# pierric/smart-chess-rust

Hardware: AMD Instinct MI355X
Metric: MCTS simulations/sec (whole node), self-play rollout=180, at 1/2/4/8 MI355X (higher is better)
Workload: dtype bf16

## Files before the change

### smart-chess-rust_amd/csrc/nn_tower32.hpp

```cpp
#pragma once
#include <type_traits>

#include "nn_kernels.hpp"

namespace scnn {

typedef __attribute__((ext_vector_type(16))) float f32x16;
typedef __attribute__((ext_vector_type(8))) int i32x8;

struct PrecBF16 {
    static constexpr bool FP8 = false;
    static constexpr int EB = 2;
    static constexpr int KS = 16;
    static constexpr int FB = 16;
    typedef bf16x8 frag;
};
struct PrecFP8 {
    static constexpr bool FP8 = true;
    static constexpr int EB = 1;
    static constexpr int KS = 64;
    static constexpr int FB = 32;
    typedef i32x8 frag;
};
template <class P>
constexpr int pix_stride(int channels) { return channels * P::EB + 16; }

template <class P>
__device__ __forceinline__ typename P::frag lds_frag_p(int byte_off) {
    if constexpr (P::FP8) {
        typedef __attribute__((ext_vector_type(4))) int i32x4;
        const i32x4 a = *reinterpret_cast<const i32x4*>(g_smem + byte_off), b = *reinterpret_cast<const i32x4*>(g_smem + byte_off + 16);
        return i32x8{a[0], a[1], a[2], a[3], b[0], b[1], b[2], b[3]};
    } else {
        return lds_frag(byte_off);
    }
}
template <class P>
__device__ __forceinline__ typename P::frag wload_p(__amdgpu_buffer_rsrc_t rsrc, int voff, int ct, int soff) {
    if constexpr (P::FP8) {
        const bf16x8 a = wload(rsrc, voff + ct * 2048, soff), b = wload(rsrc, voff + ct * 2048 + 1024, soff);
        typedef __attribute__((ext_vector_type(4))) int i32x4;
        const i32x4 x = __builtin_bit_cast(i32x4, a), y = __builtin_bit_cast(i32x4, b);
        return i32x8{x[0], x[1], x[2], x[3], y[0], y[1], y[2], y[3]};
    } else {
        return wload(rsrc, voff + ct * 1024, soff);
    }
}
template <class P>
__device__ __forceinline__ f32x16 mma_p(const typename P::frag& a, const typename P::frag& b, const f32x16& c, int scale_a) {
    if constexpr (P::FP8) return __builtin_amdgcn_mfma_scale_f32_32x32x64_f8f6f4(a, b, c, 0, 0, 0, scale_a, 0, 127);
    else return __builtin_amdgcn_mfma_f32_32x32x16_bf16(a, b, c, 0, 0, 0);
}
__device__ __forceinline__ uint32_t pk_fp8x4(float a, float b, float c, float d) {
    int w = __builtin_amdgcn_cvt_pk_fp8_f32(a, b, 0, false);
    return (uint32_t)__builtin_amdgcn_cvt_pk_fp8_f32(c, d, w, true);
}

__device__ inline int gpix2board(int pt, int i) {
    const bool inA = (i < 4) || (i >= 12 && i < 16) || (i >= 20 && i < 28);
    const int a = inA ? (i < 4 ? i : (i < 16 ? i - 8 : i - 12)) : (i < 12 ? i - 4 : (i < 20 ? i - 8 : i - 16));
    return ((2 * pt + (inA ? 0 : 1) + 4 * (a >> 3)) << 3) | (a & 7);
}

typedef float f32x2 __attribute__((ext_vector_type(2)));
typedef __bf16 bf16pair __attribute__((ext_vector_type(2)));
typedef short s16x2 __attribute__((ext_vector_type(2)));
template <typename V>
__device__ __forceinline__ f32x2 pair(const V& v, int k) { return f32x2{v[k], v[k + 1]}; }
__device__ __forceinline__ f32x2 splat(float x) { return f32x2{x, x}; }
__device__ __forceinline__ uint32_t pk_bf16(f32x2 y) { return __builtin_bit_cast(uint32_t, __builtin_convertvector(y, bf16pair)); }
__device__ __forceinline__ uint32_t pk_bf16_relu(f32x2 y) {
    s16x2 s = __builtin_bit_cast(s16x2, __builtin_convertvector(y, bf16pair));
    return __builtin_bit_cast(uint32_t, __builtin_elementwise_max(s, s16x2{0, 0}));
}

template <class P, bool RELU>
__device__ __forceinline__ void store4(int byte_off_row, int chan, f32x2 lo, f32x2 hi) {
    if constexpr (P::FP8) {
        const float l = RELU ? 0.f : -448.f;
        *reinterpret_cast<uint32_t*>(g_smem + byte_off_row + chan) =
            pk_fp8x4(__builtin_amdgcn_fmed3f(lo.x, l, 448.f), __builtin_amdgcn_fmed3f(lo.y, l, 448.f),
                     __builtin_amdgcn_fmed3f(hi.x, l, 448.f), __builtin_amdgcn_fmed3f(hi.y, l, 448.f));
    } else {
        *reinterpret_cast<uint2*>(g_smem + byte_off_row + chan * 2) =
            RELU ? make_uint2(pk_bf16_relu(lo), pk_bf16_relu(hi)) : make_uint2(pk_bf16(lo), pk_bf16(hi));
    }
}

template <int CT>
__device__ __forceinline__ int chan32(int wave, int ct, int g, int h) { return wave * (32 * CT) + ct * 32 + 8 * g + 4 * h; }

template <int CT>
struct ChP {
    f32x4 v[CT][4];
};
template <int CT>
__device__ __forceinline__ void ch_load(ChP<CT>& P, const float* __restrict__ p, int wave, int h) {
#pragma unroll
    for (int ct = 0; ct < CT; ct++)
#pragma unroll
        for (int g = 0; g < 4; g++) P.v[ct][g] = *reinterpret_cast<const f32x4*>(p + chan32<CT>(wave, ct, g, h));
}
template <int CT>
__device__ __forceinline__ void ch_load_lds(ChP<CT>& P, int byte_off, int wave, int h) {
#pragma unroll
    for (int ct = 0; ct < CT; ct++)
#pragma unroll
        for (int g = 0; g < 4; g++) P.v[ct][g] = *reinterpret_cast<const f32x4*>(g_smem + byte_off + chan32<CT>(wave, ct, g, h) * 4);
}
template <int CT>
__device__ __forceinline__ void acc_init(f32x16 (&acc)[CT][2], const ChP<CT>& B) {
#pragma unroll
    for (int ct = 0; ct < CT; ct++)
#pragma unroll
        for (int pt = 0; pt < 2; pt++)
#pragma unroll
            for (int r = 0; r < 16; r++) acc[ct][pt][r] = B.v[ct][r >> 2][r & 3];
}

#ifndef SC_T32_AB
#define SC_T32_AB 4
#endif
template <class P, int CIN, int TAPS, int CT, int TILES, int PSB, int RS, int TPI, bool PRE, int AB = SC_T32_AB>
__device__ __forceinline__ void conv_mma32(int xoff, const bf16_t* __restrict__ Wp, int wave_u, int lane, const int (&px)[2],
                                           f32x16 (&acc)[CT][2], typename P::frag (&bq)[RS][CT], int next_first, const int (&sa)[CT]) {
    typedef typename P::frag frag;
    constexpr int KPT = CIN / P::KS;
    constexpr int SPG = KPT * TPI;
    constexpr int NG = TAPS / TPI;
    constexpr int TB = 64 * P::FB;
    constexpr int SBB = TILES * TB;
    constexpr int KSB = P::KS * P::EB;
    constexpr int PD = RS - 1, AD = AB - 1;
    static_assert(TAPS % TPI == 0 && SPG % RS == 0 && PD < SPG, "bad ring / tap-group geometry");
    static_assert(SPG % AB == 0 && AD <= SPG, "bad image buffer geometry");
    const __amdgpu_buffer_rsrc_t rsrc = __builtin_amdgcn_make_buffer_rsrc(
        const_cast<bf16_t*>(Wp) + (size_t)wave_u * CT * (TB / 2), 0, 0x7fffffff, 0x00020000);
    const int voff = lane * 16;
    auto toffb = [](int t) { return (TAPS == 9) ? ((((t * 11) >> 5) - 1) * 10 + (t - 3 * ((t * 11) >> 5)) - 1) * PSB : 0; };
    frag xq[AB][2];
    int wcur = 0;
    int pc[TPI][2];
#pragma unroll
    for (int tl = 0; tl < TPI; tl++)
#pragma unroll
        for (int pt = 0; pt < 2; pt++) pc[tl][pt] = xoff + px[pt] + toffb(tl);
    if (!PRE) {
#pragma unroll
        for (int st = 0; st < PD; st++)
#pragma unroll
            for (int ct = 0; ct < CT; ct++) bq[st][ct] = wload_p<P>(rsrc, voff, ct, st * SBB);
    }
#pragma unroll
    for (int v = 0; v < AD; v++)
#pragma unroll
        for (int pt = 0; pt < 2; pt++) xq[v][pt] = lds_frag_p<P>(pc[v / KPT][pt] + (v % KPT) * KSB);
#pragma unroll 1
    for (int j = 0; j < NG; j++) {
        const int tn = (j + 1 == NG) ? 0 : j + 1;
        const int wnext = (j == NG - 1) ? next_first : tn * (SPG * SBB);
        int pn[TPI][2];
#pragma unroll
        for (int tl = 0; tl < TPI; tl++)
#pragma unroll
            for (int pt = 0; pt < 2; pt++) pn[tl][pt] = xoff + px[pt] + toffb(tn * TPI + tl);
#pragma unroll
        for (int u = 0; u < SPG; u++) {
            const int slot = u % RS;
#pragma unroll
            for (int ct = 0; ct < CT; ct++)
                bq[(slot + PD) % RS][ct] = (u + PD < SPG) ? wload_p<P>(rsrc, voff, ct, wcur + (u + PD) * SBB)
                                                          : wload_p<P>(rsrc, voff, ct, wnext + (u + PD - SPG) * SBB);
#pragma unroll
            for (int pt = 0; pt < 2; pt++) {
                const int v = u + AD;
                xq[v % AB][pt] = (v < SPG) ? lds_frag_p<P>(pc[v / KPT][pt] + (v % KPT) * KSB)
                                           : lds_frag_p<P>(pn[(v - SPG) / KPT][pt] + ((v - SPG) % KPT) * KSB);
            }
#pragma unroll
            for (int ct = 0; ct < CT; ct++)
#pragma unroll
                for (int pt = 0; pt < 2; pt++)
                    acc[ct][pt] = mma_p<P>(bq[slot][ct], xq[u % AB][pt], acc[ct][pt], sa[ct]);
#pragma unroll
            for (int m = 0; m < 2 * CT; m++) {
                __builtin_amdgcn_sched_group_barrier(0x008, 1, 0);
                if (P::FP8) {
                    __builtin_amdgcn_sched_group_barrier(0x100, CT == 1 ? 2 : 1, 0);
                    __builtin_amdgcn_sched_group_barrier(0x020, 1, 0);
                } else if (CT == 1) {
                    __builtin_amdgcn_sched_group_barrier(0x100, 1, 0);
                    if (m == 0) __builtin_amdgcn_sched_group_barrier(0x020, 1, 0);
                } else {
                    if ((m & 1) == 0)
                        __builtin_amdgcn_sched_group_barrier(0x100, 1, 0);
                    else
                        __builtin_amdgcn_sched_group_barrier(0x020, 1, 0);
                }
            }
            __builtin_amdgcn_sched_barrier(0);
        }
        wcur = wnext;
#pragma unroll
        for (int tl = 0; tl < TPI; tl++)
#pragma unroll
            for (int pt = 0; pt < 2; pt++) pc[tl][pt] = pn[tl][pt];
    }
}

struct LnStat {
    float rstd[2], nm[2];
};
template <int CT>
__device__ inline void ln_reduce(const f32x16 (&acc)[CT][2], LnStat& L, int count, int wave, int lane, float* s_stat2,
                                 int& parity, int& bad) {
    float2* st = reinterpret_cast<float2*>(s_stat2) + (parity & 1) * 256;
    parity ^= 1;
    const int i = lane & 31;
    float s[2], q[2];
#pragma unroll
    for (int pt = 0; pt < 2; pt++) {
        f32x2 a2 = {0.f, 0.f}, b2 = {0.f, 0.f};
#pragma unroll
        for (int ct = 0; ct < CT; ct++)
#pragma unroll
            for (int r = 0; r < 16; r += 2) {
                const f32x2 v = pair(acc[ct][pt], r);
                a2 += v;
                b2 = v * v + b2;
            }
        s[pt] = a2.x + a2.y;
        q[pt] = b2.x + b2.y;
    }
    {
        const auto rs = __builtin_amdgcn_permlane32_swap(__float_as_uint(s[0]), __float_as_uint(s[1]), false, false);
        const auto rq = __builtin_amdgcn_permlane32_swap(__float_as_uint(q[0]), __float_as_uint(q[1]), false, false);
        st[wave * 64 + lane] = make_float2(__uint_as_float(rs[0]) + __uint_as_float(rs[1]), __uint_as_float(rq[0]) + __uint_as_float(rq[1]));
    }
    __syncthreads();
    const float inv = 1.0f / (float)count;
#pragma unroll
    for (int pt = 0; pt < 2; pt++) {
        const int gp = pt * 32 + i;
        float2 a0 = st[gp], a1 = st[64 + gp], a2 = st[128 + gp], a3 = st[192 + gp];
        float S = (a0.x + a1.x) + (a2.x + a3.x);
        float Q = (a0.y + a1.y) + (a2.y + a3.y);
        float mean = S * inv;
        float var = Q * inv - mean * mean;
        bad |= (var != var) ? 1 : 0;
        var = fmaxf(var, 0.f);
        L.rstd[pt] = __frsqrt_rn(var + 1e-6f);
        L.nm[pt] = -mean * L.rstd[pt];
    }
}
template <int CT>
__device__ __forceinline__ void ln_apply(f32x16 (&acc)[CT][2], const LnStat& L, const ChP<CT>& G, const ChP<CT>& E, bool relu) {
#pragma unroll
    for (int pt = 0; pt < 2; pt++)
#pragma unroll
        for (int ct = 0; ct < CT; ct++)
#pragma unroll
            for (int r = 0; r < 16; r += 2) {
                const f32x2 t = pair(acc[ct][pt], r) * splat(L.rstd[pt]) + splat(L.nm[pt]);
                const f32x2 y = t * pair(G.v[ct][r >> 2], r & 3) + pair(E.v[ct][r >> 2], r & 3);
                acc[ct][pt][r] = relu ? fmaxf(y.x, 0.f) : y.x;
                acc[ct][pt][r + 1] = relu ? fmaxf(y.y, 0.f) : y.y;
            }
}
template <class P, int CT>
__device__ __forceinline__ void ln_apply_relu_store(const f32x16 (&acc)[CT][2], const LnStat& L, const ChP<CT>& G, const ChP<CT>& E,
                                                    const int (&pixbase)[2], int wave, int h) {
#pragma unroll
    for (int ct = 0; ct < CT; ct++)
#pragma unroll
        for (int pt = 0; pt < 2; pt++)
#pragma unroll
            for (int g = 0; g < 4; g++) {
                f32x2 y[2];
#pragma unroll
                for (int hf = 0; hf < 2; hf++) {
                    const f32x2 t = pair(acc[ct][pt], 4 * g + 2 * hf) * splat(L.rstd[pt]) + splat(L.nm[pt]);
                    y[hf] = t * pair(G.v[ct][g], 2 * hf) + pair(E.v[ct][g], 2 * hf);
                }
                store4<P, true>(pixbase[pt], chan32<CT>(wave, ct, g, h), y[0], y[1]);
            }
}
template <int CT>
__device__ inline void layernorm32(f32x16 (&acc)[CT][2], const ChP<CT>& G, const ChP<CT>& E, int count, bool relu, int wave,
                                   int lane, float* s_stat2, int& parity, int& bad) {
    LnStat L;
    ln_reduce<CT>(acc, L, count, wave, lane, s_stat2, parity, bad);
    ln_apply<CT>(acc, L, G, E, relu);
}

template <class P, int CT>
__device__ inline void store_image32(const f32x16 (&acc)[CT][2], const int (&pixbase)[2], int wave, int h) {
#pragma unroll
    for (int ct = 0; ct < CT; ct++)
#pragma unroll
        for (int pt = 0; pt < 2; pt++)
#pragma unroll
            for (int g = 0; g < 4; g++)
                store4<P, false>(pixbase[pt], chan32<CT>(wave, ct, g, h), pair(acc[ct][pt], 4 * g), pair(acc[ct][pt], 4 * g + 2));
}

template <int CTRL>
__device__ __forceinline__ float dpp_mov(float x) { return dpp_f<CTRL>(x); }
template <int LVL>
__device__ __forceinline__ float pool_xchg(float x) {
    if constexpr (LVL == 1) return dpp_mov<0x140>(x);
    else if constexpr (LVL == 2) return dpp_mov<0x141>(x);
    else if constexpr (LVL == 3) return dpp_mov<0x4E>(x);
    else return dpp_mov<0xB1>(x);
}
template <int NV, int W, int LVL>
__device__ __forceinline__ void pool_level(float (&v)[NV], int lane) {
    if constexpr (LVL < 5) {
        if constexpr (W >= 1) {
            if constexpr (LVL == 0) {
#pragma unroll
                for (int t = 0; t < W; t++) {
                    const auto r = __builtin_amdgcn_permlane16_swap(__float_as_uint(v[t]), __float_as_uint(v[t + W]), false, false);
                    v[t] = __uint_as_float(r[0]) + __uint_as_float(r[1]);
                }
            } else {
                const bool hi = (lane & (16 >> LVL)) != 0;
#pragma unroll
                for (int t = 0; t < W; t++) {
                    float send = hi ? v[t] : v[t + W], keep = hi ? v[t + W] : v[t];
                    v[t] = keep + pool_xchg<LVL>(send);
                }
            }
            pool_level<NV, W / 2, LVL + 1>(v, lane);
        } else {
            v[0] += pool_xchg<LVL>(v[0]);
            pool_level<NV, 0, LVL + 1>(v, lane);
        }
    }
}

template <class P, int CT, int TILES, int RS>
__device__ __forceinline__ void ring_fill(typename P::frag (&bq)[RS][CT], const bf16_t* __restrict__ Wp, int wave_u, int lane) {
    constexpr int TB = 64 * P::FB;
    const __amdgpu_buffer_rsrc_t rsrc = __builtin_amdgcn_make_buffer_rsrc(
        const_cast<bf16_t*>(Wp) + (size_t)wave_u * CT * (TB / 2), 0, 0x7fffffff, 0x00020000);
#pragma unroll
    for (int st = 0; st < RS - 1; st++)
#pragma unroll
        for (int ct = 0; ct < CT; ct++) bq[st][ct] = wload_p<P>(rsrc, lane * 16, ct, st * TILES * TB);
}
template <class P, int CT>
__device__ __forceinline__ void scale_load(int (&sa)[CT], const NetDev& net, int conv_idx, int wave, int lane) {
#pragma unroll
    for (int ct = 0; ct < CT; ct++)
        sa[ct] = P::FP8 ? __builtin_bit_cast(int, net.wf[net.f_scales + (size_t)((conv_idx * 8 + wave * CT + ct) * 64 + lane)]) : 127;
}

template <class P, int C>
struct TowerLds {
    static constexpr int IMG_BYTES = (100 * pix_stride<P>(C) > 4864 * 4) ? 100 * pix_stride<P>(C) : 4864 * 4;
    static constexpr int HIMG_BYTES = 64 * pix_stride<P>(HEAD);
    static constexpr int HIMG = IMG_BYTES;
    static constexpr int STAT = HIMG + HIMG_BYTES;
    static constexpr int VEC = STAT + 4096;
    static constexpr int SCL = VEC + 3072;
    static constexpr int RED = SCL + 1024;
    static constexpr int PAR = RED + 64;
    static constexpr int TOTAL = PAR + 15 * C * 2;
    static_assert(4864 * 4 <= IMG_BYTES, "policy logits (and the softmax pass that reads 19 x 256 of them) must fit in the image area");
    static_assert(IMG_BYTES % 16 == 0 && HIMG_BYTES % 16 == 0, "LDS regions must stay 16-byte aligned");
    static_assert(6 * HEAD * 4 + 3 * POL_PAD * 4 <= TOTAL - VEC, "head parameters must fit in the staging area");
};
static_assert(TowerLds<PrecBF16, 128>::TOTAL == 73088 && TowerLds<PrecBF16, 256>::TOTAL == 102528, "bf16 tower LDS");
static_assert(TowerLds<PrecFP8, 128>::TOTAL == 48960 && TowerLds<PrecFP8, 256>::TOTAL == 60544, "fp8 tower LDS");

struct NoPre {
    __device__ __forceinline__ bool operator()(int) const { return true; }
};
struct Fc1Hand {
    typedef __attribute__((ext_vector_type(4))) unsigned int u32x4;
    Fc1W w;
    uint32_t early;
    int have_a;
    u32x4 a[8];
};
struct NoHand {};
template <class P, int C, int RS, int TPI, int AB = SC_T32_AB, class Pre = NoPre, class Hand = NoHand>
__device__ __forceinline__ bool tower_body(const TowerArgs& A, const int pos, const int8_t* planes_lds, Pre pre, Hand& fhr) {
    constexpr bool FUSED = !std::is_same<Pre, NoPre>::value;
    constexpr bool HAND = std::is_same<Hand, Fc1Hand>::value;
    Hand* const fh = &fhr;
    typedef typename P::frag frag;
    constexpr int CT = C / 128;
    constexpr int TILES = C / 32;
    constexpr int PSB = pix_stride<P>(C);
    constexpr int HPSB = pix_stride<P>(HEAD);
    constexpr int EB = P::EB;
    constexpr int HRS = P::FP8 ? C / 64 : 8, HAB = P::FP8 ? 2 : SC_T32_AB;
    constexpr int H2RS = P::FP8 ? HEAD / 64 : 16, H2AB = P::FP8 ? 2 : SC_T32_AB;
    constexpr int NTW = C / 64;
    typedef TowerLds<P, C> Lds;
    unsigned char* smem = g_smem;
    float* s_stat = reinterpret_cast<float*>(smem + Lds::STAT);
    float* s_scl = reinterpret_cast<float*>(smem + Lds::SCL);
    float* s_red = reinterpret_cast<float*>(smem + Lds::RED);
    bf16_t* s_xb = reinterpret_cast<bf16_t*>(smem + Lds::VEC);
    float* s_z = reinterpret_cast<float*>(smem);

    const int tid = threadIdx.x, lane = tid & 63;
    const int wave = __builtin_amdgcn_readfirstlane(tid >> 6);
    const int i32 = lane & 31, h = lane >> 5;
    const NetDev& net = A.net;
    const int bp[2] = {gpix2board(0, i32), gpix2board(1, i32)};
    const int pixbase[2] = {hidx(bp[0]) * PSB, hidx(bp[1]) * PSB};
    const int px[2] = {pixbase[0] + h * P::FB, pixbase[1] + h * P::FB};

    frag ring[RS][CT];
    int sa[CT], san[CT];
    scale_load<P, CT>(sa, net, 0, wave, lane);
    scale_load<P, CT>(san, net, net.n_blocks > 0 ? 1 : 1 + 2 * net.n_blocks, wave, lane);
    ChP<CT> Bn;
    const int p_in = tid >> 2, q_in = tid & 3;
    uint32_t win[7];
    if (!FUSED && !planes_lds) {
        const uint32_t* src = reinterpret_cast<const uint32_t*>(A.boards + (size_t)pos * 7168 + p_in * 112 + q_in * 28);
#pragma unroll
        for (int k = 0; k < 7; k++) win[k] = src[k];
    }
    static_assert(C <= 256, "one parameter vector per thread");
    f32x4 spv = f32x4{0.f, 0.f, 0.f, 0.f};
    if (tid < 3 * C / 4) spv = *reinterpret_cast<const f32x4*>(net.wf + net.f_stem + tid * 4);
    else if (tid < C) spv = *reinterpret_cast<const f32x4*>(net.wf + net.f_blocks + (tid - 3 * C / 4) * 4);
    if (!FUSED || wave != 0) ring_fill<P, CT, TILES, RS>(ring, net.wb + net.o_stem, wave, lane);
    __builtin_amdgcn_sched_barrier(0);
    if constexpr (FUSED) {
        __shared__ int s_go;
        if (wave <= 1) {
            const bool go = pre(wave);
            if (wave == 0 && lane == 0) s_go = go ? 1 : 0;
            if (wave == 0) ring_fill<P, CT, TILES, RS>(ring, net.wb + net.o_stem, wave, lane);
        } else {
            uint4* z = reinterpret_cast<uint4*>(smem);
            for (int k = tid - 128; k < 100 * PSB / 16; k += 128) z[k] = make_uint4(0, 0, 0, 0);
        }
        __syncthreads();
        if (!s_go) return false;
    } else {
        uint4* z = reinterpret_cast<uint4*>(smem);
        for (int k = tid; k < 100 * PSB / 16; k += 256) z[k] = make_uint4(0, 0, 0, 0);
        __syncthreads();
    }
    if (FUSED || planes_lds) {
        const uint32_t* src = reinterpret_cast<const uint32_t*>(planes_lds + p_in * 112 + q_in * 28);
#pragma unroll
        for (int k = 0; k < 7; k++) win[k] = src[k];
    }
    {
        uint32_t* dst = reinterpret_cast<uint32_t*>(smem + hidx(p_in) * PSB + q_in * 28 * EB);
#pragma unroll
        for (int k = 0; k < 7; k++) {
            const uint32_t w = win[k];
            float v[4];
#pragma unroll
            for (int b = 0; b < 4; b++) v[b] = (float)(int8_t)((w >> (8 * b)) & 0xff);
            if constexpr (P::FP8) {
                dst[k] = pk_fp8x4(v[0], v[1], v[2], v[3]);
            } else {
                dst[2 * k] = pk_bf16(f32x2{v[0], v[1]});
                dst[2 * k + 1] = pk_bf16(f32x2{v[2], v[3]});
            }
        }
        if (tid < C) *reinterpret_cast<f32x4*>(g_smem + Lds::PAR + tid * 16) = spv;
    }
    __syncthreads();

    f32x16 acc[CT][2];
    int ln_parity = 0;
    int bad = 0;
    f32x16 res[CT][2];
    auto store_res = [&]() {
#pragma unroll
        for (int ct = 0; ct < CT; ct++)
#pragma unroll
            for (int pt = 0; pt < 2; pt++) res[ct][pt] = acc[ct][pt];
    };
    auto dump = [&](int stage) {
        if constexpr (FUSED) return;
        if (A.dbg && A.dbg_stage == stage) {
#pragma unroll
            for (int ct = 0; ct < CT; ct++)
#pragma unroll
                for (int pt = 0; pt < 2; pt++)
#pragma unroll
                    for (int r = 0; r < 16; r++)
                        A.dbg[((size_t)pos * 64 + bp[pt]) * C + chan32<CT>(wave, ct, r >> 2, h) + (r & 3)] = acc[ct][pt][r];
        }
    };

    {
        ch_load_lds<CT>(Bn, Lds::PAR, wave, h);
        acc_init<CT>(acc, Bn);
        const bf16_t* w0 = net.wb + net.o_stem;
        conv_mma32<P, 128, 9, CT, TILES, PSB, RS, TPI, true, AB>(0, w0, wave, lane, px, acc, ring, (int)((net.wb + net.o_blocks) - w0) * 2, sa);
        ChP<CT> G, E;
        ch_load_lds<CT>(G, Lds::PAR + C * 4, wave, h);
        ch_load_lds<CT>(E, Lds::PAR + 2 * C * 4, wave, h);
        ch_load_lds<CT>(Bn, Lds::PAR + 3 * C * 4, wave, h);
        layernorm32<CT>(acc, G, E, C, true, wave, lane, s_stat, ln_parity, bad);
    }
    store_res();
    store_image32<P, CT>(acc, pixbase, wave, h);
    __syncthreads();
    dump(0);
    const int head_conv0 = 1 + 2 * net.n_blocks;

#pragma unroll 1
    for (int b = 0; b < net.n_blocks; b++) {
        const bf16_t* wb = net.wb + net.o_blocks + (size_t)b * net.blk_stride_b;
        const float* wf = net.wf + net.f_blocks + (size_t)b * net.blk_stride_f;
        constexpr int NT1 = C / 32;
        constexpr int NTW1 = NT1 / 4;
        constexpr int PAR_V4 = 15 * C / 8;
        constexpr int NPV = (PAR_V4 + 255) / 256;
        constexpr int P_G1 = Lds::PAR, P_E1 = Lds::PAR + 4 * C, P_B2 = Lds::PAR + 8 * C, P_G2 = Lds::PAR + 12 * C, P_E2 = Lds::PAR + 16 * C;
        constexpr int P_SB1 = Lds::PAR + 20 * C, P_SB2 = Lds::PAR + 22 * C, P_BN = Lds::PAR + 26 * C;
        f32x4 pv[NPV];
#pragma unroll
        for (int k = 0; k < NPV; k++)
            if (tid + 256 * k < PAR_V4) pv[k] = *reinterpret_cast<const f32x4*>(wf + C + (size_t)(tid + 256 * k) * 4);
        __builtin_amdgcn_sched_barrier(0);
        acc_init<CT>(acc, Bn);
#pragma unroll
        for (int ct = 0; ct < CT; ct++) sa[ct] = san[ct];
        scale_load<P, CT>(san, net, 2 + 2 * b, wave, lane);
        conv_mma32<P, C, 9, CT, TILES, PSB, RS, TPI, true, AB>(0, wb, wave, lane, px, acc, ring, 9 * C * C * EB, sa);
#pragma unroll
        for (int k = 0; k < NPV; k++)
            if (tid + 256 * k < PAR_V4) *reinterpret_cast<f32x4*>(g_smem + Lds::PAR + (tid + 256 * k) * 16) = pv[k];
        {
            LnStat L;
            ln_reduce<CT>(acc, L, C, wave, lane, s_stat, ln_parity, bad);
            ChP<CT> G, E;
            ch_load_lds<CT>(G, P_G1, wave, h);
            ch_load_lds<CT>(E, P_E1, wave, h);
            ln_apply_relu_store<P, CT>(acc, L, G, E, pixbase, wave, h);
        }
        ch_load_lds<CT>(Bn, P_B2, wave, h);
        __syncthreads();
        acc_init<CT>(acc, Bn);
        {
            const int nxt = (b + 1 < net.n_blocks) ? (int)(net.blk_stride_b * 2 - (size_t)9 * C * C * EB) : 0;
#pragma unroll
            for (int ct = 0; ct < CT; ct++) sa[ct] = san[ct];
            scale_load<P, CT>(san, net, b + 1 < net.n_blocks ? 3 + 2 * b : head_conv0, wave, lane);
            conv_mma32<P, C, 9, CT, TILES, PSB, RS, TPI, true, AB>(0, wb + (size_t)9 * C * C * EB / 2, wave, lane, px, acc, ring, nxt, sa);
        }
        VecW<C, NTW1> w1;
        VecW<C / 2, NTW> w2;
        vec_w_load<C, NTW1, NT1>(w1, wb + (size_t)9 * C * C * EB, wave * NTW1, lane);
        vec_w_load<C / 2, NTW, C / 16>(w2, wb + (size_t)9 * C * C * EB + (size_t)C * (C / 2), wave * NTW, lane);
        __builtin_amdgcn_sched_barrier(0);
        {
            LnStat L;
            ln_reduce<CT>(acc, L, C, wave, lane, s_stat, ln_parity, bad);
            ChP<CT> G, E;
            ch_load_lds<CT>(G, P_G2, wave, h);
            ch_load_lds<CT>(E, P_E2, wave, h);
            ln_apply<CT>(acc, L, G, E, false);
        }
        {
            constexpr int NV = 16 * CT;
            float v[NV];
#pragma unroll
            for (int ct = 0; ct < CT; ct++)
#pragma unroll
                for (int r = 0; r < 16; r += 2) {
                    const f32x2 t = pair(acc[ct][0], r) + pair(acc[ct][1], r);
                    v[ct * 16 + r] = t.x;
                    v[ct * 16 + r + 1] = t.y;
                }
            pool_level<NV, NV / 2, 0>(v, lane);
            const int idx = (NV == 32) ? i32 : (i32 >> 1);
            s_xb[chan32<CT>(wave, idx >> 4, (idx & 15) >> 2, h) + (idx & 3)] = f2bf(v[0] * (1.0f / 64.0f));
        }
        float sb1[NTW1], sb2[NTW];
#pragma unroll
        for (int k = 0; k < NTW1; k++) sb1[k] = *reinterpret_cast<const float*>(g_smem + P_SB1 + (wave * (16 * NTW1) + (lane & 15) * NTW1 + k) * 4);
#pragma unroll
        for (int k = 0; k < NTW; k++) sb2[k] = *reinterpret_cast<const float*>(g_smem + P_SB2 + (chan0<NTW>(wave, lane) + k) * 4);
        __syncthreads();
        bf16_t* s_hid = s_xb + 256;
        {
            f32x4 hh[NTW1];
#pragma unroll
            for (int k = 0; k < NTW1; k++) hh[k] = f32x4{0.f, 0.f, 0.f, 0.f};
            vec_mma<C, NTW1>(s_xb, w1, lane, hh);
            if (lane < 16) {
#pragma unroll
                for (int k = 0; k < NTW1; k++) {
                    const int j = wave * (16 * NTW1) + (lane & 15) * NTW1 + k;
                    float t = hh[k][0] + sb1[k];
                    s_hid[j] = f2bf(fmaxf(t, 0.f));
                }
            }
        }
        __syncthreads();
        {
            f32x4 sc[NTW];
#pragma unroll
            for (int k = 0; k < NTW; k++) sc[k] = f32x4{0.f, 0.f, 0.f, 0.f};
            vec_mma<C / 2, NTW>(s_hid, w2, lane, sc);
            if (lane < 16) {
                const int c0 = chan0<NTW>(wave, lane);
#pragma unroll
                for (int k = 0; k < NTW; k++)
                    s_scl[c0 + k] = __builtin_amdgcn_rcpf(1.0f + __expf(-(sc[k][0] + sb2[k])));
            }
        }
#pragma unroll
        for (int ct = 0; ct < CT; ct++)
#pragma unroll
            for (int g = 0; g < 4; g++) {
                const int ch = chan32<CT>(wave, ct, g, h);
                const f32x4 sv = *reinterpret_cast<const f32x4*>(s_scl + ch);
#pragma unroll
                for (int pt = 0; pt < 2; pt++) {
                    const f32x4 rv = f32x4{res[ct][pt][4 * g], res[ct][pt][4 * g + 1], res[ct][pt][4 * g + 2], res[ct][pt][4 * g + 3]};
#pragma unroll
                    for (int k = 0; k < 4; k += 2) {
                        const f32x2 y = pair(acc[ct][pt], 4 * g + k) * pair(sv, k) + pair(rv, k);
                        acc[ct][pt][4 * g + k] = fmaxf(y.x, 0.f);
                        acc[ct][pt][4 * g + k + 1] = fmaxf(y.y, 0.f);
                    }
                }
            }
        store_res();
        store_image32<P, CT>(acc, pixbase, wave, h);
        ch_load_lds<CT>(Bn, P_BN, wave, h);
        __syncthreads();
        dump(b + 1);
    }
    dump(1000);

    const int gpb[2] = {i32 * HPSB, (32 + i32) * HPSB};
    constexpr int HP_V = Lds::VEC, HP_P1 = Lds::VEC + 3 * HEAD * 4, HP_P2 = Lds::VEC + 6 * HEAD * 4;
    f32x4 hpv[2];
#pragma unroll
    for (int k = 0; k < 2; k++)
        if (tid + 256 * k < 480) hpv[k] = *reinterpret_cast<const f32x4*>(net.wf + net.f_vhead + (size_t)(tid + 256 * k) * 4);
    __builtin_amdgcn_sched_barrier(0);
    frag hr[HRS][2];
    frag hr2[H2RS][1];
    int sh[2], sh2[1];
    scale_load<P, 2>(sh, net, head_conv0, wave, lane);
    {
        f32x16 hv[2][2];
#pragma unroll
        for (int ct = 0; ct < 2; ct++)
#pragma unroll
            for (int pt = 0; pt < 2; pt++)
#pragma unroll
                for (int r = 0; r < 16; r++) hv[ct][pt][r] = 0.f;
        conv_mma32<P, C, 1, 2, 8, PSB, HRS, 1, false, HAB>(0, net.wb + net.o_vconv, wave, lane, px, hv, hr,
                                                           (int)((net.wb + net.o_pconv1) - (net.wb + net.o_vconv)) * 2, sh);
        scale_load<P, 2>(sh, net, head_conv0 + 1, wave, lane);
        scale_load<P, 1>(sh2, net, head_conv0 + 2, wave, lane);
#pragma unroll
        for (int k = 0; k < 2; k++)
            if (tid + 256 * k < 480) *reinterpret_cast<f32x4*>(g_smem + Lds::VEC + (tid + 256 * k) * 16) = hpv[k];
        __builtin_amdgcn_sched_barrier(0);
        __syncthreads();
        ChP<2> Bv, G, E;
        ch_load_lds<2>(Bv, HP_V, wave, h);
#pragma unroll
        for (int ct = 0; ct < 2; ct++)
#pragma unroll
            for (int pt = 0; pt < 2; pt++)
#pragma unroll
                for (int r = 0; r < 16; r++) hv[ct][pt][r] += Bv.v[ct][r >> 2][r & 3];
        LnStat L;
        int badv = bad;
        ln_reduce<2>(hv, L, HEAD, wave, lane, s_stat, ln_parity, badv);
        ch_load_lds<2>(G, HP_V + HEAD * 4, wave, h);
        ch_load_lds<2>(E, HP_V + 2 * HEAD * 4, wave, h);
        ln_apply<2>(hv, L, G, E, true);
        const __amdgpu_buffer_rsrc_t hrs = __builtin_amdgcn_make_buffer_rsrc(A.hval + (size_t)pos * (64 * HEAD), 0, 0x7fffffff, 0x00020000);
        const bool wt = HAND && A.fc1_arrive;
#pragma unroll
        for (int ct = 0; ct < 2; ct++)
#pragma unroll
            for (int pt = 0; pt < 2; pt++) {
                const int off = (((wave * 2 + ct) * 2 + pt) * 64 + lane) * 32;
#pragma unroll
                for (int q = 0; q < 2; q++) {
                    typedef __attribute__((ext_vector_type(4))) unsigned int u32x4;
                    u32x4 v = {pk_bf16(pair(hv[ct][pt], 8 * q)), pk_bf16(pair(hv[ct][pt], 8 * q + 2)), pk_bf16(pair(hv[ct][pt], 8 * q + 4)),
                               pk_bf16(pair(hv[ct][pt], 8 * q + 6))};
                    if (badv) v = u32x4{0x7fc07fc0u, 0x7fc07fc0u, 0x7fc07fc0u, 0x7fc07fc0u};
                    if (wt) __builtin_amdgcn_raw_buffer_store_b128(v, hrs, off + 16 * q, 0, AUX_SC1);
                    else __builtin_amdgcn_raw_buffer_store_b128(v, hrs, off + 16 * q, 0, 0);
                }
            }
    }
    {
        ChP<2> Bv, G, E;
        ch_load_lds<2>(Bv, HP_P1, wave, h);
        f32x16 hp[2][2];
        acc_init<2>(hp, Bv);
        conv_mma32<P, C, 1, 2, 8, PSB, HRS, 1, true, HAB>(0, net.wb + net.o_pconv1, wave, lane, px, hp, hr, 0, sh);
        if (HAND && A.fc1_arrive) asm volatile("s_waitcnt vmcnt(0)" ::: "memory");
        ring_fill<P, 1, 4, H2RS>(hr2, net.wb + net.o_pconv2, wave, lane);
        __builtin_amdgcn_sched_barrier(0);
        LnStat L;
        ln_reduce<2>(hp, L, HEAD, wave, lane, s_stat, ln_parity, bad);
        if (HAND && A.fc1_arrive && tid == 0)
            __hip_atomic_fetch_add(A.fc1_arrive + (pos >> 6) * 32, 1u, __ATOMIC_RELAXED, __HIP_MEMORY_SCOPE_AGENT);
        ch_load_lds<2>(G, HP_P1 + HEAD * 4, wave, h);
        ch_load_lds<2>(E, HP_P1 + 2 * HEAD * 4, wave, h);
        ln_apply<2>(hp, L, G, E, false);
        const int xb[2] = {Lds::HIMG + gpb[0], Lds::HIMG + gpb[1]};
        store_image32<P, 2>(hp, xb, wave, h);
    }
    __syncthreads();
    {
        ChP<1> Bv, G, E;
        ch_load_lds<1>(Bv, HP_P2, wave, h);
        f32x16 z[1][2];
        acc_init<1>(z, Bv);
        const int pxh[2] = {gpb[0] + h * P::FB, gpb[1] + h * P::FB};
        conv_mma32<P, HEAD, 1, 1, 4, HPSB, H2RS, 1, true, H2AB>(Lds::HIMG, net.wb + net.o_pconv2, wave, lane, pxh, z, hr2, 0, sh2);
        uint32_t first = 0;
        if (HAND && A.fc1_arrive && tid == 0 && !A.fc1_acquire)
            first = __hip_atomic_load(A.fc1_arrive + (pos >> 6) * 32, __ATOMIC_RELAXED, __HIP_MEMORY_SCOPE_AGENT);
        LnStat L;
        ln_reduce<1>(z, L, 73, wave, lane, s_stat, ln_parity, bad);
        ch_load_lds<1>(G, HP_P2 + POL_PAD * 4, wave, h);
        ch_load_lds<1>(E, HP_P2 + 2 * POL_PAD * 4, wave, h);
        ln_apply<1>(z, L, G, E, false);
        __syncthreads();
#pragma unroll
        for (int pt = 0; pt < 2; pt++)
#pragma unroll
            for (int r = 0; r < 16; r++) {
                const int ch = chan32<1>(wave, 0, r >> 2, h) + (r & 3);
                if (ch < 73) s_z[ch * 64 + bp[pt]] = z[0][pt][r];
            }
        if (bad) s_z[lane] = __builtin_nanf("");
        if (HAND && A.fc1_arrive && tid == 0) reinterpret_cast<int*>(s_red)[8] = !A.fc1_acquire && (int32_t)(first - A.fc1_target) >= 0;
    }
    __syncthreads();
    if constexpr (HAND) {
        if (A.fc1_arrive) {
            fc1_wload(fh->w, net, pos & 63, 64, wave, lane);
            fh->have_a = reinterpret_cast<const int*>(s_red)[8];
            if (fh->have_a) fc1_load_a(fh->a, A.hval, pos >> 6, pos & 63, tid);
            else if (tid == 0) fh->early = __hip_atomic_load(A.fc1_arrive + (pos >> 6) * 32, __ATOMIC_RELAXED, __HIP_MEMORY_SCOPE_AGENT);
        }
    }
    float zv[19];
#pragma unroll
    for (int j = 0; j < 19; j++) {
        const float t = s_z[tid + 256 * j];
        zv[j] = (tid + 256 * j < 4672) ? t : -3.0e38f;
    }
    float mw = zv[0];
#pragma unroll
    for (int j = 1; j < 19; j++) mw = fmaxf(mw, zv[j]);
    mw = wave_max_fixed(mw);
    float sw = 0.f;
#pragma unroll
    for (int j = 0; j < 19; j++) sw += __expf(zv[j] - mw);
    sw = wave_sum_fixed(sw);
    if (lane == 0) {
        s_red[wave] = mw;
        s_red[4 + wave] = sw;
    }
    __syncthreads();
    const float mx = fmaxf(fmaxf(s_red[0], s_red[1]), fmaxf(s_red[2], s_red[3]));
    const float se = (s_red[4] * __expf(s_red[0] - mx) + s_red[5] * __expf(s_red[1] - mx)) +
                     (s_red[6] * __expf(s_red[2] - mx) + s_red[7] * __expf(s_red[3] - mx));
    const float lse = mx + __logf(se);
    if (A.logp) {
        float* lp = A.logp + (size_t)pos * 4672;
#pragma unroll
        for (int j = 0; j < 19; j++)
            if (tid + 256 * j < 4672) lp[tid + 256 * j] = zv[j] - lse;
    }
    if (A.prior) {
        const int n = A.n_legal[pos];
        const uint16_t* li = A.legal_idx + (size_t)pos * 224;
        float e = 0.f;
        if (tid < n) e = __expf(s_z[li[tid]] - lse);
        float s = e;
        s = wave_sum_fixed(s);
        __syncthreads();
        if (lane == 0) s_red[wave] = s;
        __syncthreads();
        s = (s_red[0] + s_red[1]) + (s_red[2] + s_red[3]) + 1e-5f;
        if (tid < n) A.prior[(size_t)pos * 224 + tid] = e / s;
    }
    return true;
}

}
```

### smart-chess-rust_amd/csrc/step_kernels.hip

```cpp
#include "search_expand.hpp"
#include "nn_kernels.hpp"
#include "nn_tower32.hpp"

#include "launchers.hpp"
#include "tower_config.hpp"

namespace scstep {

__device__ __forceinline__ void fc1_tail(const scnn::TowerArgs& A, const sc::SpParams& p, const int g, const bool ran, scnn::Fc1Hand& fh) {
    const int tid = threadIdx.x, lane = tid & 63;
    const int wave = __builtin_amdgcn_readfirstlane(tid >> 6);
    const int mb = g >> 6, ks = g & 63;
    uint32_t* ctr = A.fc1_arrive + mb * 32;
    if (!ran) {
        if (tid == 0) __hip_atomic_fetch_add(ctr, 1u, __ATOMIC_RELAXED, __HIP_MEMORY_SCOPE_AGENT);
        scnn::fc1_wload(fh.w, A.net, ks, 64, wave, lane);
        __builtin_amdgcn_sched_barrier(0);
    }
    const scnn::Fc1W& w = fh.w;
    const bool have_a = ran && fh.have_a;
    if (tid == 0 && !have_a) {
        const uint64_t t0 = __builtin_amdgcn_s_memrealtime();
        uint32_t seen = ran ? fh.early : __hip_atomic_load(ctr, __ATOMIC_RELAXED, __HIP_MEMORY_SCOPE_AGENT);
        while ((int32_t)(seen - A.fc1_target) < 0) {
            __builtin_amdgcn_s_sleep(4);
            const uint64_t waited = __builtin_amdgcn_s_memrealtime() - t0;
            if (waited > 20000000ull) {
                atomicOr(&p.cnt->err, sc::ERR_HANDOFF_TIMEOUT);
                break;
            }
            if (waited > 100000ull && (__hip_atomic_load(&p.cnt->err, __ATOMIC_RELAXED, __HIP_MEMORY_SCOPE_AGENT) & sc::ERR_HANDOFF_TIMEOUT)) break;
            seen = __hip_atomic_load(ctr, __ATOMIC_RELAXED, __HIP_MEMORY_SCOPE_AGENT);
        }
        if (A.fc1_acquire) __builtin_amdgcn_fence(__ATOMIC_ACQUIRE, "agent");
        asm volatile("s_waitcnt vmcnt(0)" ::: "memory");
    }
    __syncthreads();
    scnn::bf16_t* s_a = reinterpret_cast<scnn::bf16_t*>(scnn::g_smem);
    if (!have_a) scnn::fc1_load_a(fh.a, A.hval, mb, ks, tid);
    scnn::fc1_put_a(s_a, fh.a, tid);
    __syncthreads();
    scnn::fc1_mma_store(w, s_a, A.vpart, A.n_pos, mb, ks, 64, wave, lane);
}

template <class P, int C, int RS, int TPI, int AB, bool STAMPS = false>
__global__ __launch_bounds__(256, 1) void k_step(scnn::TowerArgs A, sc::SpParams p, int do_expand) {
    __shared__ __attribute__((aligned(16))) int8_t s_stage[7168];
    __shared__ sc::move_t s_moves[sc::MAXC];
    __shared__ sc::Position s_pos;
    __shared__ sc::Position s_hist[8];
    __shared__ uint16_t s_ps[sc::DEPTH_LDS];
    __shared__ sc::HelperBox s_box;
    const int g = blockIdx.x;
    const int lane = threadIdx.x & 63;
    scnn::kernarg_prefetch<sizeof(scnn::TowerArgs) + sizeof(sc::SpParams) + sizeof(int)>();
#define PHASE_STAMP(k, cond) do { if constexpr (STAMPS) { if (p.dbg_cycles && (cond)) p.dbg_cycles[(size_t)g * 32 + (k)] = __builtin_amdgcn_s_memrealtime(); } } while (0)
    PHASE_STAMP(24, threadIdx.x == 0);
    if (threadIdx.x == 0) s_box.state = 0;
    __syncthreads();
    auto search = [&](int wave) -> bool {
        if (wave == 1) {
            sc::dev_encode_helper(p, g, lane, &s_box, s_stage, &s_pos, s_ps, s_hist);
            return true;
        }
        constexpr bool SC_ST = STAMPS;
        SC_STAMP(0);
        sc::GameCtl cs_pre{};
        bool cs_pre_valid = false;
        if (do_expand) {
            sc::dev_expand<SC_ST>(p, g, lane, &s_pos, cs_pre, cs_pre_valid);
            __builtin_amdgcn_wave_barrier();
        }
        SC_STAMP(1);
        const bool need_net = sc::dev_select<false, SC_ST>(p, g, lane, s_stage, s_moves, &s_pos, s_ps, s_hist, cs_pre, cs_pre_valid, &s_box);
        PHASE_STAMP(25, lane == 0);
        return need_net;
    };
    scnn::Fc1Hand fh;
    const bool ran = scnn::tower_body<P, C, RS, TPI, AB>(A, g, s_stage, search, fh);
    PHASE_STAMP(26, threadIdx.x == 0);
    if (A.fc1_arrive) fc1_tail(A, p, g, ran, fh);
    PHASE_STAMP(27, threadIdx.x == 0);
#undef PHASE_STAMP
}

}

namespace scl {
template <class T, bool STAMPS = false>
constexpr auto step_kernel(T) { return &scstep::k_step<typename T::P, T::C, T::RS, T::TPI, T::AB, STAMPS>; }

const char* step_init() {
    for (bool fp8 : {false, true})
        for (int C : {128, 256}) {
            const hipError_t e = scnn::with_tower_cfg(fp8, C, [](auto cfg) {
                return hipFuncSetAttribute(reinterpret_cast<const void*>(step_kernel(cfg)), hipFuncAttributeMaxDynamicSharedMemorySize, cfg.LDS_BYTES);
            });
            if (e != hipSuccess) return hipGetErrorString(e);
        }
    const hipError_t e = hipFuncSetAttribute(reinterpret_cast<const void*>(step_kernel<scnn::TowerBf16N, true>({})), hipFuncAttributeMaxDynamicSharedMemorySize,
                                             scnn::TowerBf16N::LDS_BYTES);
    return e == hipSuccess ? nullptr : hipGetErrorString(e);
}
int step_blocks_per_cu(const scnn::NetLayout& net) {
    int n = 0;
    const hipError_t e = scnn::with_tower_cfg(net.fp8, net.C, [&](auto cfg) {
        return hipOccupancyMaxActiveBlocksPerMultiprocessor(&n, step_kernel(cfg), 256, cfg.LDS_BYTES);
    });
    return e == hipSuccess && n > 0 ? n : 1;
}
void step(const scnn::TowerArgs& a, const sc::SpParams& p, int do_expand, hipStream_t s) {
    const dim3 grid(p.n_slots), block(256);
    if (!a.net.fp8 && a.net.C == 128 && p.dbg_cycles)
        hipLaunchKernelGGL((step_kernel<scnn::TowerBf16N, true>({})), grid, block, scnn::TowerBf16N::LDS_BYTES, s, a, p, do_expand);
    else
        scnn::with_tower_cfg(a.net.fp8, a.net.C, [&](auto cfg) { hipLaunchKernelGGL(step_kernel(cfg), grid, block, cfg.LDS_BYTES, s, a, p, do_expand); });
}
}
```

Measured before the change: 2.303 million.

## Run search wave first, hoist tower prologue loads, prefetch legal-move gather

Wave 0 now runs the MCTS select/expand callback before any tower prologue work. The stem ring fill and parameter-vector loads that used to sit in front of it are issued afterwards, with wave 2 loading wave 0's parameter slice. The callback is specialized per wave through compile-time constants and reads SpParams straight from the kernarg segment to cut register pressure. In bf16, the legal-move count and index gather are issued before the final policy conv so their global latency overlaps the MMA. The cost is more reordering complexity and extra registers held live across the conv.

```diff
diff --git a/smart-chess-rust_amd/csrc/nn_tower32.hpp b/smart-chess-rust_amd/csrc/nn_tower32.hpp
--- a/smart-chess-rust_amd/csrc/nn_tower32.hpp
+++ b/smart-chess-rust_amd/csrc/nn_tower32.hpp
@@ -374,8 +374,11 @@
 static_assert(TowerLds<PrecBF16, 128>::TOTAL == 73088 && TowerLds<PrecBF16, 256>::TOTAL == 102528, "bf16 tower LDS");
 static_assert(TowerLds<PrecFP8, 128>::TOTAL == 48960 && TowerLds<PrecFP8, 256>::TOTAL == 60544, "fp8 tower LDS");
 
+template <int W>
+using WaveC = std::integral_constant<int, W>;
 struct NoPre {
-    __device__ __forceinline__ bool operator()(int) const { return true; }
+    template <class W>
+    __device__ __forceinline__ bool operator()(W) const { return true; }
 };
 struct Fc1Hand {
     typedef __attribute__((ext_vector_type(4))) unsigned int u32x4;
@@ -411,12 +414,22 @@
     const int wave = __builtin_amdgcn_readfirstlane(tid >> 6);
     const int i32 = lane & 31, h = lane >> 5;
     const NetDev& net = A.net;
-    const int bp[2] = {gpix2board(0, i32), gpix2board(1, i32)};
-    const int pixbase[2] = {hidx(bp[0]) * PSB, hidx(bp[1]) * PSB};
-    const int px[2] = {pixbase[0] + h * P::FB, pixbase[1] + h * P::FB};
-
+    int bp[2], pixbase[2], px[2];
     frag ring[RS][CT];
     int sa[CT], san[CT];
+    __shared__ int s_go;
+    if constexpr (FUSED) {
+        if (wave == 0) {
+            const bool go = pre(WaveC<0>());
+            if (lane == 0) s_go = go ? 1 : 0;
+        }
+    }
+#pragma unroll
+    for (int t = 0; t < 2; t++) {
+        bp[t] = gpix2board(t, i32);
+        pixbase[t] = hidx(bp[t]) * PSB;
+        px[t] = pixbase[t] + h * P::FB;
+    }
     scale_load<P, CT>(sa, net, 0, wave, lane);
     scale_load<P, CT>(san, net, net.n_blocks > 0 ? 1 : 1 + 2 * net.n_blocks, wave, lane);
     ChP<CT> Bn;
@@ -428,18 +441,19 @@
         for (int k = 0; k < 7; k++) win[k] = src[k];
     }
     static_assert(C <= 256, "one parameter vector per thread");
-    f32x4 spv = f32x4{0.f, 0.f, 0.f, 0.f};
-    if (tid < 3 * C / 4) spv = *reinterpret_cast<const f32x4*>(net.wf + net.f_stem + tid * 4);
-    else if (tid < C) spv = *reinterpret_cast<const f32x4*>(net.wf + net.f_blocks + (tid - 3 * C / 4) * 4);
-    if (!FUSED || wave != 0) ring_fill<P, CT, TILES, RS>(ring, net.wb + net.o_stem, wave, lane);
+    auto par_vec = [&](int v) {
+        return *reinterpret_cast<const f32x4*>(net.wf + (v < 3 * C / 4 ? net.f_stem + v * 4 : net.f_blocks + (v - 3 * C / 4) * 4));
+    };
+    const bool own_par = !(FUSED && wave == 0) && tid < C, w0_par = FUSED && wave == 2;
+    f32x4 spv = f32x4{0.f, 0.f, 0.f, 0.f}, spv0 = f32x4{0.f, 0.f, 0.f, 0.f};
+    if (own_par) spv = par_vec(tid);
+    if (w0_par) spv0 = par_vec(lane);
+    ring_fill<P, CT, TILES, RS>(ring, net.wb + net.o_stem, wave, lane);
     __builtin_amdgcn_sched_barrier(0);
     if constexpr (FUSED) {
-        __shared__ int s_go;
-        if (wave <= 1) {
-            const bool go = pre(wave);
-            if (wave == 0 && lane == 0) s_go = go ? 1 : 0;
-            if (wave == 0) ring_fill<P, CT, TILES, RS>(ring, net.wb + net.o_stem, wave, lane);
-        } else {
+        if (wave == 1) {
+            pre(WaveC<1>());
+        } else if (wave >= 2) {
             uint4* z = reinterpret_cast<uint4*>(smem);
             for (int k = tid - 128; k < 100 * PSB / 16; k += 128) z[k] = make_uint4(0, 0, 0, 0);
         }
@@ -470,7 +484,8 @@
                 dst[2 * k + 1] = pk_bf16(f32x2{v[2], v[3]});
             }
         }
-        if (tid < C) *reinterpret_cast<f32x4*>(g_smem + Lds::PAR + tid * 16) = spv;
+        if (own_par) *reinterpret_cast<f32x4*>(g_smem + Lds::PAR + tid * 16) = spv;
+        if (w0_par) *reinterpret_cast<f32x4*>(g_smem + Lds::PAR + lane * 16) = spv0;
     }
     __syncthreads();
 
@@ -722,12 +737,20 @@
         store_image32<P, 2>(hp, xb, wave, h);
     }
     __syncthreads();
+    constexpr bool GATHER_EARLY = !P::FP8;
+    int g_n = 0;
+    uint16_t g_li = 0;
     {
         ChP<1> Bv, G, E;
         ch_load_lds<1>(Bv, HP_P2, wave, h);
         f32x16 z[1][2];
         acc_init<1>(z, Bv);
         const int pxh[2] = {gpb[0] + h * P::FB, gpb[1] + h * P::FB};
+        if (GATHER_EARLY && A.prior) {
+            g_n = A.n_legal[pos];
+            g_li = A.legal_idx[(size_t)pos * 224 + (tid < 223 ? tid : 223)];
+            __builtin_amdgcn_sched_barrier(0);
+        }
         conv_mma32<P, HEAD, 1, 1, 4, HPSB, H2RS, 1, true, H2AB>(Lds::HIMG, net.wb + net.o_pconv2, wave, lane, pxh, z, hr2, 0, sh2);
         uint32_t first = 0;
         if (HAND && A.fc1_arrive && tid == 0 && !A.fc1_acquire)
@@ -787,10 +810,10 @@
             if (tid + 256 * j < 4672) lp[tid + 256 * j] = zv[j] - lse;
     }
     if (A.prior) {
-        const int n = A.n_legal[pos];
         const uint16_t* li = A.legal_idx + (size_t)pos * 224;
+        const int n = GATHER_EARLY ? g_n : A.n_legal[pos];
         float e = 0.f;
-        if (tid < n) e = __expf(s_z[li[tid]] - lse);
+        if (tid < n) e = __expf(s_z[GATHER_EARLY ? g_li : li[tid]] - lse);
         float s = e;
         s = wave_sum_fixed(s);
         __syncthreads();
diff --git a/smart-chess-rust_amd/csrc/step_kernels.hip b/smart-chess-rust_amd/csrc/step_kernels.hip
--- a/smart-chess-rust_amd/csrc/step_kernels.hip
+++ b/smart-chess-rust_amd/csrc/step_kernels.hip
@@ -58,23 +58,32 @@
     PHASE_STAMP(24, threadIdx.x == 0);
     if (threadIdx.x == 0) s_box.state = 0;
     __syncthreads();
-    auto search = [&](int wave) -> bool {
-        if (wave == 1) {
+    auto search = [&](auto wave_c) -> bool {
+        constexpr int wave = decltype(wave_c)::value;
+        if constexpr (wave == 1) {
             sc::dev_encode_helper(p, g, lane, &s_box, s_stage, &s_pos, s_ps, s_hist);
             return true;
+        } else {
+            static_assert(sizeof(scnn::TowerArgs) % 8 == 0 && sizeof(sc::SpParams) % 8 == 0, "the argument block is packed: A, p, do_expand");
+            unsigned long long ka = (unsigned long long)__builtin_amdgcn_kernarg_segment_ptr();
+            asm volatile("" : "+s"(ka));
+            typedef const __attribute__((address_space(4))) sc::SpParams* sp_kptr;
+            typedef const __attribute__((address_space(4))) int* int_kptr;
+            sc::SpParams& p = *(sc::SpParams*)(sp_kptr)(ka + sizeof(scnn::TowerArgs));
+            const int do_expand = *(int_kptr)(ka + sizeof(scnn::TowerArgs) + sizeof(sc::SpParams));
+            constexpr bool SC_ST = STAMPS;
+            SC_STAMP(0);
+            sc::GameCtl cs_pre{};
+            bool cs_pre_valid = false;
+            if (do_expand) {
+                sc::dev_expand<SC_ST>(p, g, lane, &s_pos, cs_pre, cs_pre_valid);
+                __builtin_amdgcn_wave_barrier();
+            }
+            SC_STAMP(1);
+            const bool need_net = sc::dev_select<false, SC_ST>(p, g, lane, s_stage, s_moves, &s_pos, s_ps, s_hist, cs_pre, cs_pre_valid, &s_box);
+            PHASE_STAMP(25, lane == 0);
+            return need_net;
         }
-        constexpr bool SC_ST = STAMPS;
-        SC_STAMP(0);
-        sc::GameCtl cs_pre{};
-        bool cs_pre_valid = false;
-        if (do_expand) {
-            sc::dev_expand<SC_ST>(p, g, lane, &s_pos, cs_pre, cs_pre_valid);
-            __builtin_amdgcn_wave_barrier();
-        }
-        SC_STAMP(1);
-        const bool need_net = sc::dev_select<false, SC_ST>(p, g, lane, s_stage, s_moves, &s_pos, s_ps, s_hist, cs_pre, cs_pre_valid, &s_box);
-        PHASE_STAMP(25, lane == 0);
-        return need_net;
     };
     scnn::Fc1Hand fh;
     const bool ran = scnn::tower_body<P, C, RS, TPI, AB>(A, g, s_stage, search, fh);
```

New measurement: 2.314 million, median of 6. Within noise of the previous version (+0.5%).
